# erlgo/openair4G

Measured on AMD Instinct MI355X. Metric: DL subframes/sec (20 MHz, 2x2, 64-QAM), higher is better.
Workload: dtype int16; 1 GPU; dlsim 20 MHz 2x2 TM3 (LARGE_CDD) 64-QAM MCS19x2CW, 2x14 IDFT-2048; config_id=C3, global_batch=8192, subframe_index=7, full_grid=False, parallelism=subframe-sharded x1

## Files before the change

### include/oai4g.h

```cpp
#ifndef OAI4G_H
#define OAI4G_H

#include <stddef.h>
#include <stdint.h>

#ifdef __cplusplus
extern "C" {
#endif

#define OAI4G_LTE_NULL 2
#define OAI4G_NSOFT 1827072
#define OAI4G_MAX_SEGMENTS 16
#define OAI4G_MAX_CHANNEL_BITS (14 * 1200 * 6)
#define OAI4G_D_BYTES (96 + 12 + 3 + 3 * 6144)
#define OAI4G_W_BYTES (3 * 6144 + 96)

enum { OAI4G_SISO = 0, OAI4G_ALAMOUTI = 1, OAI4G_LARGE_CDD = 2 };
enum { OAI4G_CYCLIC_PREFIX = 0, OAI4G_CYCLIC_SUFFIX = 1, OAI4G_ZEROS = 2, OAI4G_NONE = 3 };

typedef struct {
  uint16_t N_RB_DL;
  uint16_t Nid_cell;
  uint8_t Ncp;
  uint8_t nushift;
// ... 44 lines not shown
  uint8_t Nlayers;
  uint8_t first_layer;
} oai4g_dl_harq_t;

typedef struct {
  uint16_t rnti;
  uint8_t current_harq_pid;
  uint8_t Mdlharq;
  uint8_t Kmimo;
  int16_t sqrt_rho_a;
  int16_t sqrt_rho_b;
  oai4g_dl_harq_t *harq_processes[8];
} oai4g_dlsch_t;

int oai4g_init(void);
const char *oai4g_last_error(void);
int oai4g_device_name(char *buf, int len);

int oai4g_init_frame_parms(oai4g_frame_parms_t *fp, uint16_t N_RB_DL, uint16_t Nid_cell, uint8_t Ncp,
                           uint8_t nb_antennas_tx, uint8_t mode1_flag, uint8_t frame_type);
uint8_t oai4g_get_Qm(uint8_t mcs);
int oai4g_get_G(const oai4g_frame_parms_t *fp, uint16_t nb_rb, const uint32_t *rb_alloc, uint8_t mod_order,
                uint8_t Nl, uint8_t num_pdcch_symbols, int frame, uint8_t subframe);
uint8_t oai4g_get_Qm_ul(uint8_t mcs);
uint8_t oai4g_get_I_TBS(uint8_t mcs);
uint8_t oai4g_get_I_TBS_UL(uint8_t mcs);
uint32_t oai4g_tbs_bits(uint8_t I_TBS, uint16_t nb_rb);
uint32_t oai4g_get_TBS_DL(uint8_t mcs, uint16_t nb_rb);
uint32_t oai4g_get_TBS_UL(uint8_t mcs, uint16_t nb_rb);
oai4g_dlsch_t *oai4g_new_dlsch(uint8_t Kmimo, uint8_t Mdlharq, uint8_t N_RB_DL);
void oai4g_free_dlsch(oai4g_dlsch_t *dlsch);
uint32_t oai4g_lte_gold_generic(uint32_t *x1, uint32_t *x2, uint8_t reset);
int oai4g_qpp_fold32(uint32_t K, uint32_t *s, uint16_t *tab);

uint32_t oai4g_crc24a(const uint8_t *in, int bitlen);
uint32_t oai4g_crc24b(const uint8_t *in, int bitlen);
int oai4g_lte_segmentation(const uint8_t *input_buffer, uint8_t **output_buffers, uint32_t B, uint32_t *C,
                           uint32_t *Cplus, uint32_t *Cminus, uint32_t *Kplus, uint32_t *Kminus, uint32_t *F);
void oai4g_threegpplte_turbo_encoder(const uint8_t *input, uint16_t input_length_bytes, uint8_t *output,
                                     uint8_t F, uint16_t interleaver_f1, uint16_t interleaver_f2);
uint32_t oai4g_sub_block_interleaving_turbo(uint32_t D, uint8_t *d, uint8_t *w);
uint32_t oai4g_lte_rate_matching_turbo(uint32_t RTC, uint32_t G, const uint8_t *w, uint8_t *e, uint8_t C,
                                       uint32_t Nsoft, uint8_t Mdlharq, uint8_t Kmimo, uint8_t rvidx,
                                       uint8_t Qm, uint8_t Nl, uint8_t r, uint8_t nb_rb, uint8_t m);
int oai4g_dlsch_encoding(uint8_t *a, const oai4g_frame_parms_t *frame_parms, uint8_t num_pdcch_symbols,
                         oai4g_dlsch_t *dlsch, int frame, uint8_t subframe);
void oai4g_dlsch_scrambling(const oai4g_frame_parms_t *frame_parms, int mbsfn_flag, oai4g_dlsch_t *dlsch, int G,
                            uint8_t q, uint8_t Ns);
int oai4g_dlsch_modulation(int32_t **txdataF, int16_t amp, uint32_t subframe_offset,
                           const oai4g_frame_parms_t *frame_parms, uint8_t num_pdcch_symbols,
                           oai4g_dlsch_t *dlsch0, oai4g_dlsch_t *dlsch1);
void oai4g_PHY_ofdm_mod(const int32_t *input, int32_t *output, uint8_t log2fftsize, uint8_t nb_symbols,
                        uint16_t nb_prefix_samples, int etype);
void oai4g_normal_prefix_mod(const int32_t *txdataF, int32_t *txdata, uint8_t nsymb,
                             const oai4g_frame_parms_t *frame_parms);
void oai4g_do_OFDM_mod(int32_t **txdataF, int32_t **txdata, uint32_t frame, uint16_t next_slot,
                       const oai4g_frame_parms_t *frame_parms);
void oai4g_generate_pilots(int32_t **txdataF, int16_t amp, const oai4g_frame_parms_t *frame_parms, uint16_t Ntti);
int oai4g_lte_dl_cell_spec(int32_t *output, int16_t amp, const oai4g_frame_parms_t *frame_parms, uint8_t Ns,
                           uint8_t l, uint8_t p);
int oai4g_idft(int log2n, const int16_t *x, int16_t *y, int scale);
void oai4g_idft2048(const int16_t *x, int16_t *y, int scale);
void oai4g_idft1024(const int16_t *x, int16_t *y, int scale);
void oai4g_idft512(const int16_t *x, int16_t *y, int scale);
void oai4g_idft256(const int16_t *x, int16_t *y, int scale);
void oai4g_idft128(const int16_t *x, int16_t *y, int scale);
// ... 254 lines not shown
```

### openair4g_amd/__init__.py

```python
import ctypes
import os

import numpy as np

_HERE = os.path.dirname(os.path.abspath(__file__))
LIB_PATH = os.path.join(_HERE, "lib", "libopenair4g_amd.so")

LTE_NULL = 2
NSOFT = 1827072
MAX_SEGMENTS = 16
MAX_CHANNEL_BITS = 14 * 1200 * 6
D_BYTES = 96 + 12 + 3 + 3 * 6144
W_BYTES = 3 * 6144 + 96
SISO, ALAMOUTI, LARGE_CDD = 0, 1, 2
CYCLIC_PREFIX = 0


class OAI4GError(RuntimeError):
    pass


u8p = ctypes.POINTER(ctypes.c_uint8)


# ... 264 lines not shown
                                      ctypes.POINTER(FrameParms), ctypes.c_uint8, ctypes.c_uint8, ctypes.c_uint8,
                                      ctypes.c_int, ctypes.c_int]),
    "oai4g_fep_batch": (ctypes.c_int, [ctypes.POINTER(FrameParms), ctypes.c_int, ctypes.c_int, ctypes.c_void_p,
                                       ctypes.c_void_p, ctypes.c_void_p]),
    "oai4g_tx_config_create": (ctypes.c_void_p, [ctypes.POINTER(TxParams)]),
    "oai4g_tx_config_destroy": (None, [ctypes.c_void_p]),
    "oai4g_tx_G": (ctypes.c_uint32, [ctypes.c_void_p, ctypes.c_int, ctypes.c_int]),
    "oai4g_tx_ebits_words": (ctypes.c_uint32, [ctypes.c_void_p]),
    "oai4g_tx_iq_samples": (ctypes.c_uint32, [ctypes.c_void_p]),
    "oai4g_tx_workspace_bytes": (ctypes.c_size_t, [ctypes.c_void_p, ctypes.c_int]),
    "oai4g_tx_batch": (ctypes.c_int, [ctypes.c_void_p, ctypes.c_int, ctypes.c_void_p, ctypes.c_void_p,
                                      ctypes.c_void_p, ctypes.c_void_p]),
    "oai4g_tx_batch_timed": (ctypes.c_int, [ctypes.c_void_p, ctypes.c_int, ctypes.c_void_p, ctypes.c_void_p,
                                            ctypes.c_void_p, ctypes.c_void_p, ctypes.POINTER(ctypes.c_float)]),
    "oai4g_tx_encode": (ctypes.c_int, [ctypes.c_void_p, ctypes.c_int, ctypes.c_void_p, ctypes.c_void_p,
                                       ctypes.c_void_p]),
    "oai4g_tx_modulate": (ctypes.c_int, [ctypes.c_void_p, ctypes.c_int, ctypes.c_void_p, ctypes.c_void_p,
                                         ctypes.c_void_p]),
    "oai4g_tx_mod_nosat": (ctypes.c_int, [ctypes.c_void_p]),
    "oai4g_diag_encode_phase_ms": (ctypes.c_int, [ctypes.c_void_p, ctypes.c_int, ctypes.c_void_p, ctypes.c_void_p,
                                                  ctypes.c_int, ctypes.c_int, ctypes.POINTER(ctypes.c_float)]),
    "oai4g_diag_encode_occupancy": (ctypes.c_int, [ctypes.c_void_p, ctypes.POINTER(ctypes.c_int),
                                                   ctypes.POINTER(ctypes.c_size_t)]),
    "oai4g_diag_stream": (ctypes.c_int, [ctypes.c_void_p, ctypes.c_void_p, ctypes.c_size_t, ctypes.c_int,
                                         ctypes.c_void_p]),
    "oai4g_dev_alloc": (ctypes.c_void_p, [ctypes.c_size_t]),
    "oai4g_dev_free": (None, [ctypes.c_void_p]),
    "oai4g_memcpy_h2d": (ctypes.c_int, [ctypes.c_void_p, ctypes.c_void_p, ctypes.c_size_t]),
    "oai4g_memcpy_d2h": (ctypes.c_int, [ctypes.c_void_p, ctypes.c_void_p, ctypes.c_size_t]),
    "oai4g_memset_d": (ctypes.c_int, [ctypes.c_void_p, ctypes.c_int, ctypes.c_size_t]),
    "oai4g_sync": (ctypes.c_int, []),
    "oai4g_fill_payload": (ctypes.c_int, [ctypes.c_void_p, ctypes.c_size_t, ctypes.c_uint64, ctypes.c_void_p]),
    "oai4g_qpp_fold32": (ctypes.c_int, [ctypes.c_uint32, ctypes.POINTER(ctypes.c_uint32), ctypes.c_void_p]),
}


def load_library(path=None):
    global _lib
    if _lib is not None:
        return _lib
    path = path or os.environ.get("OAI4G_LIB") or LIB_PATH
    if not os.path.exists(path):
        raise OAI4GError(f"HIP library not built: {path} (run __graft_entry__.build())")
    lib = ctypes.CDLL(path)
    for name, (res, args) in _SIGS.items():
        fn = getattr(lib, name)
        fn.restype = res
        fn.argtypes = args
    _lib = lib
    return lib


def exported_symbols():
    return sorted(_SIGS)


def lib():
    return load_library()


def init():
    L = lib()
    if L.oai4g_init() != 0:
        raise OAI4GError(L.oai4g_last_error().decode())
    return L

# ... 1025 lines not shown
```

### openair4g_amd/csrc/oai4g_encode.hip

```cpp
#include "oai4g_internal.h"

struct rsc_tables_t {
  uint8_t next[8][16];
  uint8_t par[8][16];
  uint8_t apow[8][8];
  uint32_t hz;
  uint32_t zs[8];
  uint32_t fm[3];
};

static constexpr uint8_t rsc_step_c(uint8_t u, uint8_t s, uint8_t *out)
{
  *out = (uint8_t)((u ^ (s >> 2) ^ (s >> 1)) & 1);
  return (uint8_t)((((u << 2) ^ (s >> 1)) ^ ((s >> 1) << 2) ^ (s << 2)) & 7);
}

static constexpr rsc_tables_t make_rsc_tables()
{
  rsc_tables_t t{};
  for (int s = 0; s < 8; s++)
    for (int nib = 0; nib < 16; nib++) {
      uint8_t st = (uint8_t)s, p = 0;
      for (int b = 0; b < 4; b++) {
        uint8_t o = 0;
// ... 271 lines not shown
{
  uint32_t pi = start & 0xffffu, dl = start >> 16, word = 0;
#pragma unroll
  for (int b = 0; b < 32; b++) {
    word |= __builtin_amdgcn_ubfe(sys[pi >> 5], pi & 31u, 1u) << b;
    pi += dl;
    pi = min(pi, pi - K);
    dl += d2;
    dl = min(dl, dl - K);
  }
  const uint32_t n = K - 32 * j;
  return n >= 32 ? word : word & ((1u << n) - 1u);
}

static __device__ __forceinline__ void turbo_segment(const uint32_t *in, uint32_t *par_out, uint32_t K,
                                                     uint32_t *tail_out, const enc_tabs_t *tb)
{
  const uint32_t lane = threadIdx.x & 63;
  const uint32_t nch = (K + 31) >> 5;
  const uint32_t lq = nch <= 64 ? 0 : (nch <= 128 ? 1 : 2), qp = 1u << lq;
  uint32_t u[4], v[4];
  uint32_t S = 0;
#pragma unroll
  for (int t = 0; t < 4; t++) {
    u[t] = 0;
    uint32_t j = lane * qp + t;
    if (t < (int)qp && j < nch) u[t] = in[j];
    v[t] = rsc_feedback_word(u[t]);
    if (t < (int)qp) S = tb->apow[0][S] ^ (v[t] >> 29);
  }
#pragma unroll
  for (int d = 0; d < 6; d++) {
    uint32_t other = __shfl_up(S, 1u << d, 64);
    if (lane >= (1u << d)) S ^= tb->apow[lq + d][other];
  }
  uint32_t s = __shfl_up(S, 1, 64);
  if (lane == 0) s = 0;
#pragma unroll
  for (int t = 0; t < 4; t++) {
    uint32_t j = lane * qp + t;
    if (t < (int)qp && j < nch) {
      uint32_t n = min(32u, K - 32 * j);
      uint32_t par = rsc_parity_of_feedback(v[t]) ^ tb->zs[s];
      if (n < 32) {
        par &= (1u << n) - 1u;
        for (uint32_t q = 0; q < (n >> 2); q++) s = tb->next[s][(u[t] >> (4 * q)) & 15u];
      } else {
        s = tb->apow[0][s] ^ (v[t] >> 29);
      }
      par_out[j] = par;
      if (j == nch - 1) {
        uint32_t tbits = 0;
        for (int stp = 0; stp < 3; stp++) {
          uint32_t z = ((s >> 2) ^ s) & 1u, x = (s ^ (s >> 1)) & 1u;
          s >>= 1;
          tbits |= (x << (2 * stp)) | (z << (2 * stp + 1));
        }
        *tail_out = tbits;
      }
    }
  }
}

static __device__ __forceinline__ uint32_t tail_bit(const uint32_t *tails, uint32_t r, uint32_t m)
{
  return m < 6 ? (tails[2 * r] >> m) & 1u : (tails[2 * r + 1] >> (m - 6)) & 1u;
}

static __device__ __forceinline__ uint32_t dstream_bit(const uint32_t *blk, uint32_t sw, const uint32_t *tails,
                                                       uint32_t r, uint32_t K, uint32_t s, uint32_t idx)
{
  if (idx < K) return (blk[s * sw + (idx >> 5)] >> (idx & 31)) & 1u;
  return tail_bit(tails, r, 3 * (idx - K) + s);
}

static __device__ __forceinline__ uint32_t colperm(uint32_t col) { return __builtin_bitreverse32(col) >> 27; }

struct wwalk_t {
  uint32_t p, region, col, row, which;
};

static __device__ __forceinline__ void wwalk_init(wwalk_t &w, uint32_t p, uint32_t R, uint32_t Kpi)
{
  w.p = p;
  if (p < Kpi) {
    w.region = 0; w.col = p / R; w.row = p - w.col * R; w.which = 0;
  } else {
    uint32_t q = p - Kpi;
    w.region = 1; w.col = q / (2 * R);
    uint32_t rr = q - w.col * 2 * R;
    w.row = rr >> 1; w.which = rr & 1u;
  }
}

// ... 353 lines not shown
      for (int b = 0; b < 8; b++) {
        const uint32_t e = (b & 1) ? ew[b >> 1] >> 16 : ew[b >> 1];
        const uint32_t D = *(const uint32_t *)((const uint8_t *)b8 + __builtin_amdgcn_ubfe(e, 5, 10));
        acc |= __builtin_amdgcn_alignbit(D, D, e) & (0x01010101u << b);
      }
      uint32_t a0 = acc & 0xffu, a1 = (acc >> 8) & 0xffu, a2 = (acc >> 16) & 0xffu, a3 = acc >> 24;
      const uint32_t n = Q - 8 * j;
      if (n < 8) {
        const uint32_t m = (1u << n) - 1u;
        a0 &= m; a1 &= m; a2 &= m; a3 &= m;
      }
      const bool s3 = ki ? s3b : s3a;
      const uint32_t q1 = s3 ? a3 : a1, q3 = s3 ? a1 : a3;
      uint32_t *o = ilv + (i - j);
      if ((Q & 7u) == 0) {
        uint8_t *ob = (uint8_t *)o + j;
        const uint32_t qb = Q >> 3;
        ob[0] = (uint8_t)a0; ob[qb] = (uint8_t)q1; ob[2 * qb] = (uint8_t)a2; ob[3 * qb] = (uint8_t)q3;
      } else {
        or_bits(o, 8 * j, a0);
        or_bits(o, Q + 8 * j, q1);
        or_bits(o, 2 * Q + 8 * j, a2);
        or_bits(o, 3 * Q + 8 * j, q3);
      }
    }
  }
  __syncthreads();
  if (stop_phase == 23) return;

  for (uint32_t seg = wave; seg < 2 * C; seg += nwaves) {
    const uint32_t r = seg >> 1, e = seg & 1u;
    uint32_t *blk = strm + r * 3 * sw;
    const uint32_t io = r < n0 ? r * kw0 : u0 + (r - n0) * kw1;
    turbo_segment(e ? ilv + io : blk, blk + (1 + e) * sw, r < n0 ? kk0 : kk1, &tails[2 * r + e], tabs);
  }
  __syncthreads();
  if (stop_phase <= 3) return;

  if (DEBUG) {
    for (uint32_t r = 0; r < C; r++) {
      uint32_t K = cw.K[r], R = cw.R[r], Kpi = cw.Kpi[r], ND = cw.ND[r];
      const uint32_t *blk = strm + r * 3 * sw;
      if (dbg.c)
        for (uint32_t i = tid; i < K / 8; i += nth) {
          uint32_t wv = blk[(i >> 2)];
          uint32_t byte = (wv >> (8 * (i & 3))) & 0xffu;
          dbg.c[r * (8 + 3 + 768) + i] = (uint8_t)(__builtin_bitreverse32(byte) >> 24);
        }
      if (dbg.d) {
        uint8_t *d = dbg.d + (size_t)r * OAI4G_D_BYTES;
        for (uint32_t i = tid; i < 96; i += nth) d[i] = OAI4G_LTE_NULL;
        for (uint32_t i = tid; i < 3 * K + 12; i += nth) {
          uint32_t kk = i / 3, s = i - 3 * kk;
          d[96 + i] = (uint8_t)(kk < K ? dstream_bit(blk, sw, tails, r, K, s, kk) : tail_bit(tails, r, i - 3 * K));
        }
        if (tid == 0) d[96 + 3 * (K + 4) + 2] = (uint8_t)dstream_bit(blk, sw, tails, r, K, 2, 0);
      }
      if (dbg.w) {
        uint8_t *w = dbg.w + (size_t)r * OAI4G_W_BYTES;
        for (uint32_t p = tid; p < 3 * Kpi; p += nth) {
          wwalk_t wk;
          wwalk_init(wk, p, R, Kpi);
          w[p] = wwalk_null(wk, R, ND) ? OAI4G_LTE_NULL : (uint8_t)wwalk_bit(wk, blk, sw, tails, r, K, ND, Kpi);
        }
      }
    }
    if (!dbg.e) return;
  }

  const uint32_t nd0 = __builtin_amdgcn_readfirstlane(cw.NDk[0]), nd1 = __builtin_amdgcn_readfirstlane(cw.NDk[1]);
  for (uint32_t r = tid; r < C; r += nth) {
    const uint32_t K = r < n0 ? kk0 : kk1, ND = r < n0 ? nd0 : nd1;
    uint32_t *blk = strm + r * 3 * sw;
    for (uint32_t s = 0; s < 3; s++) {
      uint32_t t4 = tail_bit(tails, r, s) | (tail_bit(tails, r, 3 + s) << 1) | (tail_bit(tails, r, 6 + s) << 2) |
                    (tail_bit(tails, r, 9 + s) << 3);
      uint32_t w0 = K >> 5, off = K & 31;
      blk[s * sw + w0] |= t4 << off;
      if (off > 28) blk[s * sw + (w0 + 1)] |= t4 >> (32 - off);
    }
    if (ND == 0) blk[2 * sw + ((K + 4) >> 5)] |= (blk[2 * sw] & 1u) << ((K + 4) & 31u);
  }
  __syncthreads();

  {
    const tp_lane_t tpl = tp_lane(tid & 31);
    const uint32_t sw3 = __builtin_amdgcn_readfirstlane(3 * sw);
    const uint32_t nt0 = __builtin_amdgcn_readfirstlane(cw.ntk[0]), nt1 = __builtin_amdgcn_readfirstlane(cw.ntk[1]);
    const uint32_t Nnn0 = __builtin_amdgcn_readfirstlane(cw.Nnnk[0]), Nnn1 = __builtin_amdgcn_readfirstlane(cw.Nnnk[1]);
    const uint32_t es = __builtin_amdgcn_readfirstlane(cw.esplit[sfi]);
    const uint32_t Elo = __builtin_amdgcn_readfirstlane(cw.E[sfi][0]), Ehi = __builtin_amdgcn_readfirstlane(cw.E[sfi][C - 1]);
    const uint32_t wrapt0 = __builtin_amdgcn_readfirstlane(cw.rm_wrapt[0]), wrapt1 = __builtin_amdgcn_readfirstlane(cw.rm_wrapt[1]);
    const bool once = Ehi <= min(Nnn0, Nnn1) && Elo <= min(Nnn0, Nnn1) && wrapt0 != ~1u && wrapt1 != ~1u;
    const uint32_t pp0 = (nt0 + 1) >> 1, pp1 = (nt1 + 1) >> 1;
    const uint32_t psplit = n0 * pp0;
    const uint32_t pm0 = ((1u << 20) + pp0 - 1) / pp0, pm1 = ((1u << 20) + pp1 - 1) / pp1;
    auto ro_of = [&](uint32_t r) { return r >= es ? es * Elo + (r - es) * Ehi : r * Elo; };
    auto pair0 = [&](uint32_t r) { return r < n0 ? r * pp0 : psplit + (r - n0) * pp1; };
    auto decode = [&](uint32_t P, uint32_t &ki, uint32_t &r, uint32_t &t0) {
      ki = P >= psplit ? 1u : 0u;
      const uint32_t PP = ki ? P - psplit : P, pp = ki ? pp1 : pp0;
      const uint32_t rr = (PP * (ki ? pm1 : pm0)) >> 20, rem = PP - rr * pp;
      r = ki ? n0 + rr : rr;
      t0 = 2 * rem;
    };
    gu32_t *gold = (gu32_t *)(c->gold_tab + (size_t)(sfi * c->n_cw + cwi) * c->ebits_words);
    uint32_t *eout = DEBUG ? nullptr : ebits + (size_t)(sf * c->n_cw + cwi) * c->ebits_words;
    uint32_t *ebuf = DEBUG ? dbg_ebuf : lds_base;
    const uint32_t hb = DEBUG ? C : (C + 1) >> 1, nhalf = DEBUG ? 1u : 2u;
    uint32_t carry = 0;
    for (uint32_t h = 0; h < nhalf; h++) {
      const uint32_t rb0 = h ? hb : 0, rb1 = h ? C : hb;
      const uint32_t eb0 = ro_of(rb0), eb1 = rb1 < C ? ro_of(rb1) : G;
      const uint32_t w0 = eb0 >> 5, nwh = ((eb1 + 31) >> 5) - w0;
      for (uint32_t i = tid; i < nwh + 1; i += nth) ebuf[i] = (i == 0 && h) ? carry : 0u;
      __syncthreads();
      const uint32_t pb = pair0(rb0), pe = pair0(rb1), bit0 = 32 * w0;
      const uint32_t *rsrc0 = &cw.rm_src[0][0][0], *rdst0 = &cw.rm_dst[0][0][0];
      auto row_of = [&](uint32_t ki, uint32_t t0) {
        return __builtin_amdgcn_readfirstlane(ki * ((OAI4G_RM_TILES + 1) * 32) + t0 * 32);
      };
      auto pair_loop = [&](auto ONCE) {
        uint32_t P = pb + wave;
        uint32_t ki = 0, r = 0, t0 = 0;
        uint32_t nsrc = 1u << 5, ndst = 0;
        if (P < pe) {
          decode(P, ki, r, t0);
          const uint32_t ro = row_of(ki, t0);
          nsrc = (rsrc0 + ro)[lane];
          ndst = (rdst0 + ro)[lane];
        }
        uint32_t bbo = 0, E = 0, rob = 0, Nnn = 0, wtc = 0, tpb = 0, rowb = 0;
        auto enter = [&](uint32_t rr, uint32_t kk) {
          bbo = __builtin_amdgcn_readfirstlane(rr * sw3);
          E = rr >= es ? Ehi : Elo;
          rob = ro_of(rr) - bit0;
          Nnn = kk ? Nnn1 : Nnn0;
          wtc = kk ? wrapt1 : wrapt0;
          tpb = 2 * (kk ? pp1 : pp0);
          rowb = kk * ((OAI4G_RM_TILES + 1) * 32);
        };
        enter(r, ki);
        for (; P < pe; P += nwaves) {
          const uint32_t src = nsrc, dst = ndst;
          uint32_t k2 = ki, r2 = r, t2 = t0 + 2 * nwaves, rowb2 = rowb;
          if (t2 >= tpb) {
            uint32_t tpb2 = tpb;
            do {
              t2 -= tpb2;
              r2++;
              k2 = r2 >= n0 ? 1u : 0u;
              tpb2 = 2 * (k2 ? pp1 : pp0);
            } while (t2 >= tpb2);
            rowb2 = k2 * ((OAI4G_RM_TILES + 1) * 32);
          }
          if (P + nwaves < pe) {
            const uint32_t ro = __builtin_amdgcn_readfirstlane(rowb2 + t2 * 32);
            nsrc = (rsrc0 + ro)[lane];
            ndst = (rdst0 + ro)[lane];
          }
          const uint32_t *bb = strm + bbo - 1;
          const uint32_t *wp = bb + ((src >> 5) & 0x7fffu);
          uint32_t y = __builtin_amdgcn_alignbit(wp[1], wp[0], src);
          y = transpose32_t<0>(y, tpl);
          y >>= (dst >> 16) & 31u;
          const uint32_t o = dst & 0xffffu, m = __builtin_amdgcn_ubfe(dst, 21, 6);
          const uint32_t ro = rob;
          if constexpr (decltype(ONCE)::value) {
            const int l = min((int)m, (int)E - (int)o);
            if (l > 0) or_bits2(ebuf, ro + o, y & (0xffffffffu >> (32 - l)));
            if (wtc - t0 < 2u) {
              asm volatile("" ::: "memory");
              if (dst & OAI4G_RM_DST_WRAP) {
                const uint32_t ma = Nnn - o;
                const uint32_t l2 = min(m - ma, E);
                or_bits2(ebuf, ro, (y >> ma) & (0xffffffffu >> (32 - l2)));
              }
            }
          } else if (m) {
            y &= 0xffffffffu >> (32 - m);
            const uint32_t ma = min(m, Nnn - o);
            for (uint32_t part = 0; part < 2; part++) {
              const uint32_t len = part ? m - ma : ma, os = part ? 0u : o;
              const uint32_t v = part ? (ma < 32 ? y >> ma : 0u) : (ma < 32 ? y & ((1u << ma) - 1u) : y);
              for (uint32_t x = os; len && x < E; x += Nnn) {
                const uint32_t l = min(len, E - x);
                or_bits(ebuf, ro + x, v & (0xffffffffu >> (32 - l)));
              }
            }
          }
          if (r2 != r) enter(r2, k2);
          ki = k2;
          r = r2;
          t0 = t2;
        }
      };
      if (once) pair_loop(std::true_type{});
      else pair_loop(std::false_type{});
      __syncthreads();
      if (DEBUG) {
        for (uint32_t k = tid; k < G; k += nth) dbg.e[k] = (uint8_t)((ebuf[k >> 5] >> (k & 31)) & 1u);
        return;
      }
      const uint32_t nst = stop_phase <= 4 ? 0u : ((h + 1 < nhalf && (eb1 & 31u)) ? nwh - 1 : nwh);
      for (uint32_t i = tid; i < nst; i += nth) {
        const uint32_t wi = w0 + i;
        uint32_t v = ebuf[i] ^ gold[wi];
        const uint32_t nb = min(32u, G - 32 * wi);
        if (nb < 32) v &= (1u << nb) - 1u;
        eout[wi] = v;
      }
      if (h + 1 < nhalf) {
        carry = (eb1 & 31u) ? ebuf[nwh - 1] : 0u;
        __syncthreads();
      }
    }
  }
}

__global__ void __launch_bounds__(256) __attribute__((amdgpu_num_sgpr(80))) k_encode(const cfg_dev_t *__restrict__ c, const uint8_t *__restrict__ payload,
                                                uint32_t *__restrict__ ebits, int stop_phase, uint32_t sf0)
{
  extern __shared__ uint32_t lds_dyn[];
  uint32_t sf = blockIdx.x / c->n_cw, cwi = blockIdx.x % c->n_cw;
  enc_debug_t none = {nullptr, nullptr, nullptr, nullptr, nullptr};
  encode_codeword<false>(c, sf, cwi, payload, ebits, none, lds_dyn, stop_phase, sf0);
}
// ... 270 lines not shown
```

### openair4g_amd/csrc/oai4g_host.cpp

```cpp
#include <hip/hip_runtime.h>
#include <math.h>
#include <pthread.h>
#include <stdarg.h>
#include <stdio.h>
#include <stdlib.h>
#include <string.h>

#include <algorithm>
#include <cmath>
#include <cstdlib>
#include <vector>
#include <map>
#include <mutex>
#include <vector>

#include "../../include/oai4g.h"
#include "../../include/oai4g_qpp.h"
#include "../../include/oai4g_tbs.h"
#include "oai4g_internal.h"

static thread_local char g_err[512] = "";

static void set_err(const char *fmt, ...)
{
// ... 646 lines not shown
      if (row < R) {
        const int pos = (int)(32 * row) - (int)ND + (s == 2 ? 1 : 0);
        const uint32_t wrel = (uint32_t)((int)(s * sw) + (pos >> 5) + 1);
        c.rm_src[ki][t][L] = ((uint32_t)pos & 31u) | (wrel << 5) | (s == 2 && row == R - 1 ? OAI4G_RM_SRC_LAST : 0u);
      }
      uint32_t wc = 0;
      for (int b = 0; b < 5; b++) wc |= ((L >> b) & 1u) << (4 - b);
      uint32_t b0 = 0, b1 = 0;
      for (uint32_t w2 = 0; w2 < wc; w2++) {
        uint32_t p2 = 0;
        for (int b = 0; b < 5; b++) p2 |= ((w2 >> b) & 1u) << (4 - b);
        b0 += p2 < ND ? 1u : 0u;
        b1 += p2 + 1 < ND ? 1u : 0u;
      }
      const uint32_t z0 = L < ND ? 1u : 0u, z1 = z0 + (L + 1 < ND ? 1u : 0u);
      const uint32_t zc = il ? z1 : z0;
      const uint32_t cs = il ? 32 * R - ND + 2 * wc * R - b0 - b1 : wc * R - b0;
      const uint32_t pc = il ? 32 * R + 2 * wc * R : wc * R;
      const int left = il ? 2 * ((int)R - 16 * (int)rb) : (int)R - 32 * (int)rb;
      int n = left < 32 ? left : 32;
      if (il && L == 31 && ND > 0 && left <= 32 && n) n--;
      const uint32_t z = rb ? 0u : zc, ci0 = rb ? cs + 32 * rb - zc : cs, p0 = pc + 32 * rb;
      const int m = p0 + (uint32_t)n > Ncb ? (int)Ncb - (int)(p0 + z) : n - (int)z;
      if (m <= 0) continue;
      uint32_t o = ci0 + Nnn - k0c;
      o = o >= Nnn ? o - Nnn : o;
      c.rm_dst[ki][t][L] = o | (z << 16) | ((uint32_t)m << 21) | (o + (uint32_t)m > Nnn ? OAI4G_RM_DST_WRAP : 0u);
      if (o + (uint32_t)m > Nnn) c.rm_wrapt[ki] = c.rm_wrapt[ki] == ~0u || c.rm_wrapt[ki] == t ? t : ~1u;
    }
  }
  if (getenv("OAI4G_ENC_GENERAL_RM")) c.rm_wrapt[ki] = ~1u;
}

extern "C" int oai4g_qpp_fold32(uint32_t K, uint32_t *s_out, uint16_t *tab)
{
  const int qi = oai4g_qpp_index(K);
  if (qi < 0 || oai4g_qpp_table[qi].K != K) return -1;
  if (K & 1023u) return 0;
  const uint64_t f1 = oai4g_qpp_table[qi].f1, f2 = oai4g_qpp_table[qi].f2;
  const uint32_t Q = K >> 5;
  auto pi = [&](uint64_t k) { return (uint32_t)((f1 * k + f2 * k * k) % K); };
  const uint32_t d = (pi(Q) + K - pi(0)) % K;
  if (d % Q) return 0;
  const uint32_t s = d / Q;
  if (!(s & 1u)) return 0;
  for (uint32_t k = 0; k < K; k++)
    if ((pi(k + Q) + K - pi(k)) % K != d) return 0;
  uint32_t si = 1;
  while (((si * s) & 31u) != 1u) si += 2;
  *s_out = s;
  for (uint32_t k = 0; k < Q; k++) {
    const uint32_t x = pi(k);
    tab[k] = (uint16_t)(((x % Q) << 7) | ((si * (x / Q)) & 31u));
  }
  return 1;
}

static int derive_cfg(oai4g_tx_config *cfg, const oai4g_tx_params_t *p, const uint8_t Nl[2], bool need_remap,
                      int only_sf)
{
  memset(&cfg->h, 0, sizeof(cfg->h));
  cfg->p = *p;
  oai4g_frame_parms_t &fp = cfg->fp;
  if (oai4g_init_frame_parms(&fp, p->N_RB_DL, p->Nid_cell, p->Ncp, p->nb_antennas_tx, p->mode1_flag,
                             p->frame_type) != 0)
    return -1;
// ... 178 lines not shown
      wwords += 3 * c.R[r] + 2;
      for (uint32_t rb = 0; rb < (c.R[r] + 31) / 32; rb++) c.tasks[ntask++] = (uint16_t)(r | (rb << 5));
      for (uint32_t rb = 0; rb < (c.R[r] + 15) / 16; rb++) c.tasks[ntask++] = (uint16_t)(r | (1u << 4) | (rb << 5));
    }
    c.wpk_off[C] = wwords;
    c.ntask = ntask;
    for (uint32_t r = 0; r < C; r++) {
      const uint32_t ki = r < c.n0 ? 0 : 1;
      if (c.K[r] != c.kk[ki]) { set_err("block size order"); return -1; }
      c.Rk[ki] = c.R[r]; c.NDk[ki] = c.ND[r]; c.Ncbk[ki] = c.Ncb[r]; c.Nnnk[ki] = c.Nnn[r]; c.k0ck[ki] = c.k0c[r];
    }
    for (uint32_t r = 0; r < C; r++) {
      const uint32_t ki = r < c.n0 ? 0 : 1;
      if (c.R[r] != c.Rk[ki] || c.ND[r] != c.NDk[ki] || c.Ncb[r] != c.Ncbk[ki] || c.Nnn[r] != c.Nnnk[ki] ||
          c.k0c[r] != c.k0ck[ki] || c.kidx[r] != ki) {
        set_err("per-size block geometry differs");
        return -1;
      }
    }
    if (c.n0 == 0) { c.Rk[0] = c.Rk[1]; c.NDk[0] = c.NDk[1]; c.Ncbk[0] = c.Ncbk[1]; c.Nnnk[0] = c.Nnnk[1]; c.k0ck[0] = c.k0ck[1]; }
    for (int ki = 0; ki < 2; ki++) {
      c.nullcol[ki][0] = c.nullcol[ki][1] = 0;
      for (uint32_t wc = 0; wc < 32; wc++) {
        uint32_t pc = 0;
        for (int b = 0; b < 5; b++) pc |= ((wc >> b) & 1u) << (4 - b);
        if (pc < c.NDk[ki]) c.nullcol[ki][0] |= 1u << wc;
        if (pc + 1 < c.NDk[ki]) c.nullcol[ki][1] |= 1u << wc;
      }
      c.t0k[ki] = (c.Rk[ki] + 31) / 32;
      c.ntk[ki] = c.t0k[ki] + (c.Rk[ki] + 15) / 16;
      c.ntmag[ki] = ((1u << 20) + c.ntk[ki] - 1) / c.ntk[ki];
      if (c.ntk[ki] > OAI4G_RM_TILES) { set_err("rate-matching plan: %u tiles", c.ntk[ki]); return -1; }
      rm_plan(c, ki);
    }
    max_w = wwords > max_w ? wwords : max_w;
    uint32_t tbw = (c.A_bytes + 3 + 3) / 4 + 1;
    max_tb_words = tbw > max_tb_words ? tbw : max_tb_words;
    uint32_t strw = C * 3 * c.stream_words;
    max_stream_words = strw > max_stream_words ? strw : max_stream_words;
    for (int sf = 0; sf < 10; sf++) {
      int G;
      if (fp.nb_antennas_tx == 4) {
        std::vector<uint16_t> tmp((size_t)14 * fp.ofdm_symbol_size);
        uint32_t sb[14];
        int n = build_remap(&fp, p->rb_alloc, p->num_pdcch_symbols, sf, p->mimo_mode, tmp.data(), sb, nullptr);
        G = n < 0 ? -1 : n * (int)c.Qm;
      } else {
        G = oai4g_get_G(&fp, p->nb_rb, p->rb_alloc, (uint8_t)c.Qm, Nl[cw], p->num_pdcch_symbols, 0, (uint8_t)sf);
      }
      if (G <= 0 || G > OAI4G_MAX_CHANNEL_BITS) { set_err("G=%d out of range", G); return -1; }
      c.G[sf] = (uint32_t)G;
      uint32_t Gp = (uint32_t)G / Nl[cw] / c.Qm, GpmodC = Gp % C, off = 0;
      for (uint32_t r = 0; r < C; r++) {
        uint32_t E = (r < C - GpmodC) ? Nl[cw] * c.Qm * (Gp / C) : Nl[cw] * c.Qm * ((GpmodC ? 1 : 0) + Gp / C);
        c.E[sf][r] = E;
        c.roff[sf][r] = off;
        off += E;
      }
      c.roff[sf][C] = off;
      c.esplit[sf] = C - GpmodC;
      for (int h = 0; h < 2; h++) {
        const uint32_t E = c.E[sf][h ? C - 1 : 0], w = (E + 31) / 32;
        c.ew[sf][h] = w;
        c.emag[sf][h] = w ? (uint32_t)(((1ull << 32) + w - 1) / w) : 0u;
      }
      uint32_t gw = (off + 31) / 32;
// ... 3234 lines not shown
```

### openair4g_amd/csrc/oai4g_internal.h

```cpp
#pragma once
#include <hip/hip_runtime.h>
#include <stdint.h>

#include "../../include/oai4g.h"

#define OAI4G_MAX_CB 16
#define OAI4G_MAX_NULLS 104
#define OAI4G_MAX_CHUNKS 192
#define OAI4G_MAX_TASKS (OAI4G_MAX_CB * 20)
#define OAI4G_RM_TILES 20
#define OAI4G_RM_SRC_LAST (1u << 20)
#define OAI4G_RM_DST_WRAP (1u << 27)
#define OAI4G_PIPE_MAX_CHUNKS 16
#define OAI4G_CRS_CODE 0xE000u
#define OAI4G_CTL_CODE 0xC000u
static constexpr uint32_t oai4g_mod_entry_shift(uint32_t mimo_mode, uint32_t n_ant, uint32_t log2N)
{
  return log2N != 11 ? 1u : mimo_mode == OAI4G_LARGE_CDD && n_ant == 2 ? 3u : mimo_mode == OAI4G_SISO ? 2u : 1u;
}
static constexpr uint32_t oai4g_mod_addr_mask(uint32_t shift) { return 0x7FFFu & ~((1u << shift) - 1u); }
static constexpr uint32_t oai4g_mod_sentinel(uint32_t N) { return (3u * N) / 4u; }
static constexpr bool oai4g_mod_nre_fits(uint32_t nre, uint32_t N) { return nre + 3u <= oai4g_mod_sentinel(N); }
#define OAI4G_ENC_CRC_TABLE_WORDS (256 + 256)
#define OAI4G_GOLD_LANES 256
// ... 33 lines not shown
  uint32_t kidx[OAI4G_MAX_CB];
  uint32_t wpk_off[OAI4G_MAX_CB + 1];
  uint32_t ntask;
  uint16_t tasks[OAI4G_MAX_TASKS];
  uint32_t ilv_off[OAI4G_MAX_CB + 1];
  uint32_t qpp0[2][OAI4G_MAX_CHUNKS];
  alignas(16) uint32_t qpp_tab[2][OAI4G_MAX_CHUNKS * 4];
  uint32_t qpp_f32[2];
  uint32_t qpp_s3[2];
  uint32_t n0, u0, kk[2], kw[2], kmag[2];
  uint32_t Rk[2], NDk[2], Ncbk[2], Nnnk[2], k0ck[2];
  uint32_t ntk[2], t0k[2], ntmag[2];
  uint32_t rm_wrapt[2];
  uint32_t nullcol[2][2];
  uint32_t esplit[10], ew[10][2], emag[10][2];
  uint32_t nnull[2];
  uint16_t nullpos[2][OAI4G_MAX_NULLS];
  uint32_t G[10];
  uint32_t E[10][OAI4G_MAX_CB];
  uint32_t roff[10][OAI4G_MAX_CB + 1];
  int16_t qam_a[8], qam_b[8];
  int16_t qpsk_a, qpsk_b;
  int16_t alm_qpsk[2][2];
  uint32_t stream_words;
  uint32_t crc_per_tb;
  uint32_t crc_per_cb;
  uint32_t crc_lpb;
  uint32_t crcmul_tb[8][6][16];
  uint32_t crcmul_blk[OAI4G_MAX_CB][96];
  uint32_t crc2_tb[2][8][96];
  uint32_t crc2_cb[2][2][8][96];
  uint32_t rm_src[2][OAI4G_RM_TILES + 1][32];
  uint32_t rm_dst[2][OAI4G_RM_TILES + 1][32];
};

struct cfg_dev_t {
  uint32_t N_RB_DL, N, log2N, cp0, cp, spt, nsymb, n_ant, first_carrier;
  uint32_t n_cw, mimo_mode, num_pdcch, rnti, Nid_cell, first_sf, sf_step;
  uint32_t payload_stride;
  uint32_t ebits_words;
  uint32_t lds_tb_words;
  uint32_t lds_stream_words;
  uint32_t lds_gold_words;
  uint32_t lds_w_words;
  uint32_t lds_a_words;
  uint32_t lds_b_words;
  uint32_t mod_nosat;
  uint32_t pad;
  uint32_t crctab[2][256];
  cw_dev_t cw[2];
  uint32_t symbase[10][14];
  uint32_t symnre[10][14];
  uint32_t n_cu;
  const uint16_t *remap;
  const uint16_t *remap_tm;
  uint32_t with_crs;
  uint32_t pilmask;
  uint32_t ctlmask[10];
  uint32_t ctl_on;
  const uint32_t *gold_tab;
  const uint32_t *gold_x1;
  const uint32_t *gold_x2j;
  const uint32_t *tw;
  const uint32_t *stat_tm;
  uint32_t stat_planes;
  uint32_t pad2;
// ... 221 lines not shown
```

Before: 8.822 million subframes/s.

## Precompute rate-matching pair schedule and specialize turbo encoder scan for aligned K

Replaces the per-wave on-device decoding of rate-matching tile pairs, which used division and walk-forward loops, with a host-precomputed descriptor table read through constant address space, and prefetches descriptors two iterations ahead. Adds a templated turbo segment encoder for K divisible by 32 that uses packed 4-bit state-propagation constants and ds_bpermute for the prefix scan, removing LDS table lookups. The apow scan in the generic path is made branchless. In exchange, the per-codeword config struct grows and host setup has more work and more failure paths.

```diff
diff --git a/include/oai4g.h b/include/oai4g.h
--- a/include/oai4g.h
+++ b/include/oai4g.h
@@ -100,6 +100,9 @@
 void oai4g_free_dlsch(oai4g_dlsch_t *dlsch);
 uint32_t oai4g_lte_gold_generic(uint32_t *x1, uint32_t *x2, uint8_t reset);
 int oai4g_qpp_fold32(uint32_t K, uint32_t *s, uint16_t *tab);
+int oai4g_rsc_scan_rows(uint32_t q, uint32_t rows[6]);
+int oai4g_rm_pair_schedule(uint32_t C, uint32_t n0, const uint32_t nt[2], const uint32_t wrapt[2],
+                           uint32_t *pairs, uint32_t *pair0);
 
 uint32_t oai4g_crc24a(const uint8_t *in, int bitlen);
 uint32_t oai4g_crc24b(const uint8_t *in, int bitlen);
diff --git a/openair4g_amd/__init__.py b/openair4g_amd/__init__.py
--- a/openair4g_amd/__init__.py
+++ b/openair4g_amd/__init__.py
@@ -320,6 +320,10 @@
     "oai4g_sync": (ctypes.c_int, []),
     "oai4g_fill_payload": (ctypes.c_int, [ctypes.c_void_p, ctypes.c_size_t, ctypes.c_uint64, ctypes.c_void_p]),
     "oai4g_qpp_fold32": (ctypes.c_int, [ctypes.c_uint32, ctypes.POINTER(ctypes.c_uint32), ctypes.c_void_p]),
+    "oai4g_rsc_scan_rows": (ctypes.c_int, [ctypes.c_uint32, ctypes.POINTER(ctypes.c_uint32)]),
+    "oai4g_rm_pair_schedule": (ctypes.c_int, [ctypes.c_uint32, ctypes.c_uint32, ctypes.POINTER(ctypes.c_uint32),
+                                              ctypes.POINTER(ctypes.c_uint32), ctypes.POINTER(ctypes.c_uint32),
+                                              ctypes.POINTER(ctypes.c_uint32)]),
 }
 
 
diff --git a/openair4g_amd/csrc/oai4g_encode.hip b/openair4g_amd/csrc/oai4g_encode.hip
--- a/openair4g_amd/csrc/oai4g_encode.hip
+++ b/openair4g_amd/csrc/oai4g_encode.hip
@@ -327,7 +327,9 @@
 #pragma unroll
   for (int d = 0; d < 6; d++) {
     uint32_t other = __shfl_up(S, 1u << d, 64);
-    if (lane >= (1u << d)) S ^= tb->apow[lq + d][other];
+    uint32_t ln = lane;
+    asm volatile("" : "+v"(ln));
+    S ^= tb->apow[lq + d][ln >= (1u << d) ? other : 0u];
   }
   uint32_t s = __shfl_up(S, 1, 64);
   if (lane == 0) s = 0;
@@ -355,6 +357,74 @@
       }
     }
   }
+}
+
+static constexpr uint32_t rsc_prop_packed(uint32_t n)
+{
+  uint32_t w = 0;
+  for (uint32_t s = 0; s < 8; s++) {
+    uint8_t st = (uint8_t)s;
+    for (uint32_t i = 0; i < n % 7; i++) {
+      uint8_t o = 0;
+      st = rsc_step_c(0, st, &o);
+    }
+    w |= (uint32_t)st << (4 * s);
+  }
+  return w;
+}
+static_assert(rsc_prop_packed(7) == 0x76543210u && rsc_prop_packed(1) != 0x76543210u, "RSC zero-input period");
+
+static __device__ __forceinline__ uint32_t rsc_prop(uint32_t packed, uint32_t s) { return (packed >> (4 * s)) & 7u; }
+
+extern "C" int oai4g_rsc_scan_rows(uint32_t q, uint32_t rows[6])
+{
+  if (q < 1 || q > 3) return -1;
+  for (uint32_t d = 0; d < 6; d++) rows[d] = rsc_prop_packed((32 * q) << d);
+  return 0;
+}
+
+template <int Q>
+static __device__ __forceinline__ void turbo_segment32(const uint32_t *in, uint32_t *par_out, uint32_t nch,
+                                                       uint32_t *tail_out, const enc_tabs_t *tb)
+{
+  constexpr uint32_t A1 = rsc_prop_packed(32), AQinv = rsc_prop_packed(7 - (32 * Q) % 7);
+  const uint32_t lane = threadIdx.x & 63, j0 = lane * Q, last = nch - 1;
+  uint32_t v[Q], S = 0;
+#pragma unroll
+  for (int t = 0; t < Q; t++) {
+    v[t] = rsc_feedback_word(in[min(j0 + t, last)]);
+    S = (t ? rsc_prop(A1, S) : 0u) ^ (v[t] >> 29);
+  }
+  const uint32_t Sloc = S;
+#pragma unroll
+  for (int d = 0; d < 6; d++) {
+    const uint32_t o = (uint32_t)__builtin_amdgcn_ds_bpermute((int)((lane - (1u << d)) << 2), (int)S);
+    uint32_t ln = lane;
+    asm volatile("" : "+v"(ln));
+    S ^= rsc_prop(rsc_prop_packed((32u * Q) << d), ln >= (1u << d) ? o : 0u);
+  }
+  uint32_t s = rsc_prop(AQinv, S ^ Sloc), fin = 0;
+  uint32_t par[Q];
+#pragma unroll
+  for (int t = 0; t < Q; t++) {
+    const uint32_t j = j0 + t;
+    const uint32_t p = rsc_parity_of_feedback(v[t]) ^ tb->zs[s];
+    s = rsc_prop(A1, s) ^ (v[t] >> 29);
+    par[t] = (t == 0 || j < nch) ? p : 0u;
+    fin = j == last ? s : fin;
+  }
+  uint32_t tbits = 0;
+#pragma unroll
+  for (int stp = 0; stp < 3; stp++) {
+    const uint32_t z = ((fin >> 2) ^ fin) & 1u, x = (fin ^ (fin >> 1)) & 1u;
+    fin >>= 1;
+    tbits |= (x << (2 * stp)) | (z << (2 * stp + 1));
+  }
+  if (j0 < nch) {
+#pragma unroll
+    for (int t = 0; t < Q; t++) par_out[j0 + t] = par[t];
+  }
+  if (last - j0 < (uint32_t)Q) *tail_out = tbits;
 }
 
 static __device__ __forceinline__ uint32_t tail_bit(const uint32_t *tails, uint32_t r, uint32_t m)
@@ -774,7 +844,13 @@
     const uint32_t r = seg >> 1, e = seg & 1u;
     uint32_t *blk = strm + r * 3 * sw;
     const uint32_t io = r < n0 ? r * kw0 : u0 + (r - n0) * kw1;
-    turbo_segment(e ? ilv + io : blk, blk + (1 + e) * sw, r < n0 ? kk0 : kk1, &tails[2 * r + e], tabs);
+    const uint32_t *in = e ? ilv + io : blk;
+    uint32_t *par = blk + (1 + e) * sw, *tail = &tails[2 * r + e];
+    const uint32_t K = r < n0 ? kk0 : kk1, nch = K >> 5;
+    if (K & 31u) turbo_segment(in, par, K, tail, tabs);
+    else if (nch > 128) turbo_segment32<3>(in, par, nch, tail, tabs);
+    else if (nch > 64) turbo_segment32<2>(in, par, nch, tail, tabs);
+    else turbo_segment32<1>(in, par, nch, tail, tabs);
   }
   __syncthreads();
   if (stop_phase <= 3) return;
@@ -828,24 +904,16 @@
   {
     const tp_lane_t tpl = tp_lane(tid & 31);
     const uint32_t sw3 = __builtin_amdgcn_readfirstlane(3 * sw);
-    const uint32_t nt0 = __builtin_amdgcn_readfirstlane(cw.ntk[0]), nt1 = __builtin_amdgcn_readfirstlane(cw.ntk[1]);
     const uint32_t Nnn0 = __builtin_amdgcn_readfirstlane(cw.Nnnk[0]), Nnn1 = __builtin_amdgcn_readfirstlane(cw.Nnnk[1]);
-    const uint32_t es = __builtin_amdgcn_readfirstlane(cw.esplit[sfi]);
-    const uint32_t Elo = __builtin_amdgcn_readfirstlane(cw.E[sfi][0]), Ehi = __builtin_amdgcn_readfirstlane(cw.E[sfi][C - 1]);
-    const uint32_t wrapt0 = __builtin_amdgcn_readfirstlane(cw.rm_wrapt[0]), wrapt1 = __builtin_amdgcn_readfirstlane(cw.rm_wrapt[1]);
-    const bool once = Ehi <= min(Nnn0, Nnn1) && Elo <= min(Nnn0, Nnn1) && wrapt0 != ~1u && wrapt1 != ~1u;
-    const uint32_t pp0 = (nt0 + 1) >> 1, pp1 = (nt1 + 1) >> 1;
-    const uint32_t psplit = n0 * pp0;
-    const uint32_t pm0 = ((1u << 20) + pp0 - 1) / pp0, pm1 = ((1u << 20) + pp1 - 1) / pp1;
-    auto ro_of = [&](uint32_t r) { return r >= es ? es * Elo + (r - es) * Ehi : r * Elo; };
-    auto pair0 = [&](uint32_t r) { return r < n0 ? r * pp0 : psplit + (r - n0) * pp1; };
-    auto decode = [&](uint32_t P, uint32_t &ki, uint32_t &r, uint32_t &t0) {
-      ki = P >= psplit ? 1u : 0u;
-      const uint32_t PP = ki ? P - psplit : P, pp = ki ? pp1 : pp0;
-      const uint32_t rr = (PP * (ki ? pm1 : pm0)) >> 20, rem = PP - rr * pp;
-      r = ki ? n0 + rr : rr;
-      t0 = 2 * rem;
-    };
+    bool once;
+    {
+      const uint32_t Elo = __builtin_amdgcn_readfirstlane(cw.E[sfi][0]), Ehi = __builtin_amdgcn_readfirstlane(cw.E[sfi][C - 1]);
+      const uint32_t wrapt0 = __builtin_amdgcn_readfirstlane(cw.rm_wrapt[0]), wrapt1 = __builtin_amdgcn_readfirstlane(cw.rm_wrapt[1]);
+      once = Ehi <= min(Nnn0, Nnn1) && Elo <= min(Nnn0, Nnn1) && wrapt0 != ~1u && wrapt1 != ~1u;
+    }
+    typedef const __attribute__((address_space(4))) uint32_t cu32_t;
+    cu32_t *pdesc = (cu32_t *)cw.rm_pairs, *ppair0 = (cu32_t *)cw.rm_pair0;
+    cu32_t *pE = (cu32_t *)cw.E[sfi], *proff = (cu32_t *)cw.roff[sfi];
     gu32_t *gold = (gu32_t *)(c->gold_tab + (size_t)(sfi * c->n_cw + cwi) * c->ebits_words);
     uint32_t *eout = DEBUG ? nullptr : ebits + (size_t)(sf * c->n_cw + cwi) * c->ebits_words;
     uint32_t *ebuf = DEBUG ? dbg_ebuf : lds_base;
@@ -853,88 +921,62 @@
     uint32_t carry = 0;
     for (uint32_t h = 0; h < nhalf; h++) {
       const uint32_t rb0 = h ? hb : 0, rb1 = h ? C : hb;
-      const uint32_t eb0 = ro_of(rb0), eb1 = rb1 < C ? ro_of(rb1) : G;
+      const uint32_t eb0 = proff[rb0], eb1 = rb1 < C ? proff[rb1] : G;
       const uint32_t w0 = eb0 >> 5, nwh = ((eb1 + 31) >> 5) - w0;
       for (uint32_t i = tid; i < nwh + 1; i += nth) ebuf[i] = (i == 0 && h) ? carry : 0u;
       __syncthreads();
-      const uint32_t pb = pair0(rb0), pe = pair0(rb1), bit0 = 32 * w0;
-      const uint32_t *rsrc0 = &cw.rm_src[0][0][0], *rdst0 = &cw.rm_dst[0][0][0];
-      auto row_of = [&](uint32_t ki, uint32_t t0) {
-        return __builtin_amdgcn_readfirstlane(ki * ((OAI4G_RM_TILES + 1) * 32) + t0 * 32);
-      };
+      const uint32_t pb = ppair0[rb0], pe = ppair0[rb1], bit0 = 32 * w0;
+      const char *rsrc0 = (const char *)&cw.rm_src[0][0][0], *rdst0 = (const char *)&cw.rm_dst[0][0][0];
       auto pair_loop = [&](auto ONCE) {
         uint32_t P = pb + wave;
-        uint32_t ki = 0, r = 0, t0 = 0;
-        uint32_t nsrc = 1u << 5, ndst = 0;
-        if (P < pe) {
-          decode(P, ki, r, t0);
-          const uint32_t ro = row_of(ki, t0);
-          nsrc = (rsrc0 + ro)[lane];
-          ndst = (rdst0 + ro)[lane];
-        }
-        uint32_t bbo = 0, E = 0, rob = 0, Nnn = 0, wtc = 0, tpb = 0, rowb = 0;
-        auto enter = [&](uint32_t rr, uint32_t kk) {
-          bbo = __builtin_amdgcn_readfirstlane(rr * sw3);
-          E = rr >= es ? Ehi : Elo;
-          rob = ro_of(rr) - bit0;
-          Nnn = kk ? Nnn1 : Nnn0;
-          wtc = kk ? wrapt1 : wrapt0;
-          tpb = 2 * (kk ? pp1 : pp0);
-          rowb = kk * ((OAI4G_RM_TILES + 1) * 32);
+        if (P >= pe) return;
+        const uint32_t plast = pe - 1;
+        uint32_t d = pdesc[P], dn = pdesc[min(P + nwaves, plast)];
+        uint32_t E, ro, nsrc, ndst;
+        auto fetch = [&]() {
+          E = pE[(d >> 2) & 15u];
+          ro = proff[(d >> 2) & 15u];
+          nsrc = *(const uint32_t *)(rsrc0 + ((d >> 16) + 4 * lane));
+          ndst = *(const uint32_t *)(rdst0 + ((d >> 16) + 4 * lane));
         };
-        enter(r, ki);
-        for (; P < pe; P += nwaves) {
-          const uint32_t src = nsrc, dst = ndst;
-          uint32_t k2 = ki, r2 = r, t2 = t0 + 2 * nwaves, rowb2 = rowb;
-          if (t2 >= tpb) {
-            uint32_t tpb2 = tpb;
-            do {
-              t2 -= tpb2;
-              r2++;
-              k2 = r2 >= n0 ? 1u : 0u;
-              tpb2 = 2 * (k2 ? pp1 : pp0);
-            } while (t2 >= tpb2);
-            rowb2 = k2 * ((OAI4G_RM_TILES + 1) * 32);
-          }
-          if (P + nwaves < pe) {
-            const uint32_t ro = __builtin_amdgcn_readfirstlane(rowb2 + t2 * 32);
-            nsrc = (rsrc0 + ro)[lane];
-            ndst = (rdst0 + ro)[lane];
-          }
-          const uint32_t *bb = strm + bbo - 1;
+        fetch();
+        for (;;) {
+          const uint32_t src = nsrc, dst = ndst, dc = d, Ec = E, rob = ro - bit0;
+          d = dn;
+          dn = pdesc[min(P + 2 * nwaves, plast)];
+          fetch();
+          const uint32_t *bb = (const uint32_t *)((const char *)strm + (dc & 0x3cu) * sw3) - 1;
           const uint32_t *wp = bb + ((src >> 5) & 0x7fffu);
           uint32_t y = __builtin_amdgcn_alignbit(wp[1], wp[0], src);
           y = transpose32_t<0>(y, tpl);
           y >>= (dst >> 16) & 31u;
           const uint32_t o = dst & 0xffffu, m = __builtin_amdgcn_ubfe(dst, 21, 6);
-          const uint32_t ro = rob;
           if constexpr (decltype(ONCE)::value) {
-            const int l = min((int)m, (int)E - (int)o);
-            if (l > 0) or_bits2(ebuf, ro + o, y & (0xffffffffu >> (32 - l)));
-            if (wtc - t0 < 2u) {
+            const int l = min((int)m, (int)Ec - (int)o);
+            if (l > 0) or_bits2(ebuf, rob + o, y & (0xffffffffu >> (32 - l)));
+            if (dc & 1u) {
               asm volatile("" ::: "memory");
               if (dst & OAI4G_RM_DST_WRAP) {
-                const uint32_t ma = Nnn - o;
-                const uint32_t l2 = min(m - ma, E);
-                or_bits2(ebuf, ro, (y >> ma) & (0xffffffffu >> (32 - l2)));
+                const uint32_t ma = ((dc & 2u) ? Nnn1 : Nnn0) - o;
+                const uint32_t l2 = min(m - ma, Ec);
+                or_bits2(ebuf, rob, (y >> ma) & (0xffffffffu >> (32 - l2)));
               }
             }
           } else if (m) {
+            const uint32_t Nnn = (dc & 2u) ? Nnn1 : Nnn0;
             y &= 0xffffffffu >> (32 - m);
             const uint32_t ma = min(m, Nnn - o);
             for (uint32_t part = 0; part < 2; part++) {
               const uint32_t len = part ? m - ma : ma, os = part ? 0u : o;
               const uint32_t v = part ? (ma < 32 ? y >> ma : 0u) : (ma < 32 ? y & ((1u << ma) - 1u) : y);
-              for (uint32_t x = os; len && x < E; x += Nnn) {
-                const uint32_t l = min(len, E - x);
-                or_bits(ebuf, ro + x, v & (0xffffffffu >> (32 - l)));
+              for (uint32_t x = os; len && x < Ec; x += Nnn) {
+                const uint32_t l = min(len, Ec - x);
+                or_bits(ebuf, rob + x, v & (0xffffffffu >> (32 - l)));
               }
             }
           }
-          if (r2 != r) enter(r2, k2);
-          ki = k2;
-          r = r2;
-          t0 = t2;
+          P += nwaves;
+          if (P >= pe) break;
         }
       };
       if (once) pair_loop(std::true_type{});
diff --git a/openair4g_amd/csrc/oai4g_host.cpp b/openair4g_amd/csrc/oai4g_host.cpp
--- a/openair4g_amd/csrc/oai4g_host.cpp
+++ b/openair4g_amd/csrc/oai4g_host.cpp
@@ -702,6 +702,26 @@
   if (getenv("OAI4G_ENC_GENERAL_RM")) c.rm_wrapt[ki] = ~1u;
 }
 
+extern "C" int oai4g_rm_pair_schedule(uint32_t C, uint32_t n0, const uint32_t nt[2], const uint32_t wrapt[2],
+                                      uint32_t *pairs, uint32_t *pair0)
+{
+  if (C < 1 || C > OAI4G_MAX_CB || n0 > C) return -1;
+  for (uint32_t ki = 0; ki < 2; ki++)
+    if ((ki ? n0 < C : n0 > 0) && (nt[ki] < 1 || nt[ki] > OAI4G_RM_TILES)) return -1;
+  uint32_t n = 0;
+  for (uint32_t r = 0; r < C; r++) {
+    const uint32_t ki = r >= n0 ? 1u : 0u, pp = (nt[ki] + 1) / 2;
+    pair0[r] = n;
+    for (uint32_t p = 0; p < pp; p++) {
+      const uint32_t t0 = 2 * p, row = ki * ((OAI4G_RM_TILES + 1) * 32) + t0 * 32;
+      const uint32_t wrap = wrapt[ki] - t0 < 2u ? 1u : 0u;
+      pairs[n++] = wrap | (ki << 1) | (r << 2) | ((4 * row) << 16);
+    }
+  }
+  pair0[C] = n;
+  return (int)n;
+}
+
 extern "C" int oai4g_qpp_fold32(uint32_t K, uint32_t *s_out, uint16_t *tab)
 {
   const int qi = oai4g_qpp_index(K);
@@ -946,6 +966,10 @@
       c.ntmag[ki] = ((1u << 20) + c.ntk[ki] - 1) / c.ntk[ki];
       if (c.ntk[ki] > OAI4G_RM_TILES) { set_err("rate-matching plan: %u tiles", c.ntk[ki]); return -1; }
       rm_plan(c, ki);
+    }
+    if (oai4g_rm_pair_schedule(C, c.n0, c.ntk, c.rm_wrapt, c.rm_pairs, c.rm_pair0) < 0) {
+      set_err("rate-matching pair schedule");
+      return -1;
     }
     max_w = wwords > max_w ? wwords : max_w;
     uint32_t tbw = (c.A_bytes + 3 + 3) / 4 + 1;
diff --git a/openair4g_amd/csrc/oai4g_internal.h b/openair4g_amd/csrc/oai4g_internal.h
--- a/openair4g_amd/csrc/oai4g_internal.h
+++ b/openair4g_amd/csrc/oai4g_internal.h
@@ -89,6 +89,8 @@
   uint32_t crc2_cb[2][2][8][96];
   uint32_t rm_src[2][OAI4G_RM_TILES + 1][32];
   uint32_t rm_dst[2][OAI4G_RM_TILES + 1][32];
+  uint32_t rm_pair0[OAI4G_MAX_CB + 1];
+  uint32_t rm_pairs[OAI4G_MAX_CB * ((OAI4G_RM_TILES + 1) / 2)];
 };
 
 struct cfg_dev_t {
```

Measured after the change: 9.062 million subframes/s (median of 6 runs). 2.7% higher.
